# mrottmann/DDalphaAMG

Hardware: AMD Instinct MI355X
Metric: fine_wilson_clover_gflops (higher is better)
Workload: dtype f32; 1 GPU; fine Wilson-Clover apply (d_plus_clover), 32x32x32x32 local lattice per GPU, random SU(3) gauge, csw=1.0, anti-periodic T; parallelism=single, ranks=1

## Files before the change

ddalphaamg_amd/csrc/fine_op.h:

```cpp
#pragma once
#include "common.h"
#include "geometry.h"
#include "halo.h"

namespace ddamg {

template <typename T>
struct FineOpDev {
  const T* D;
  const T* clover;
  const T* clover_inv;
  const int* nb;
  int V;
  const T* halo;
  HaloDev hd;
  const int* tile_nb;
  const unsigned short* tnb;
  const unsigned char* parity;
  const T* Dc;
  const signed char* Dsgn;
  const T* cloverc;
};

template <typename T>
class FineOp {
 public:
  FineOp() = default;

  void upload(const Geometry& g, const double* D_ref, const double* clover_ref, const Knobs& knobs, hipStream_t st);
  void shift_diagonal(const double* clover64, double diff, hipStream_t st);
  const T* clover_field() const { return clover_; }
  void scale_clover(const double* base64, double scale_even, double scale_odd, hipStream_t st);
  void apply(T* eta, const T* phi, hipStream_t st) const;
  FineOpDev<T> dev() const { return FineOpDev<T>{D_, clover_, clover_inv_, nb_, V_, halo_.recv(), halo_.dev(), tile_nb_, tnb_, parity_, Dc_, Dsgn_, Cc_}; }
  bool links_compressed() const { return Dc_ != nullptr; }
  int V() const { return V_; }
  void apply_f32in(T* eta, const float* phi, hipStream_t st) const;
  void set_comm(Comm* c) { comm_ = c; }
  void halo_exchange(const T* v, hipStream_t st) const;
  void halo_begin(const T* v, hipStream_t st) const;
  void halo_finish(hipStream_t st) const;
  bool distributed() const { return halo_.active(); }
  void hop(T* out, const T* in, int par, hipStream_t st, int post = 0, const T* a = nullptr) const;
  void oo_inv(T* out, const T* in, hipStream_t st) const;
  void parity_select(T* out, const T* a, const T* b, int keep, hipStream_t st) const;

 private:
  DeviceBuffer<T> D_, clover_, clover_inv_;
  DeviceBuffer<int> nb_;
  DeviceBuffer<int> lex_;
  DeviceBuffer<unsigned char> parity_;
  DeviceBuffer<int> tile_nb_;
  T* Dc_ = nullptr;
  DeviceBuffer<T> Dc_store_;
  DeviceBuffer<signed char> Dsgn_;
  T* Cc_ = nullptr;
  DeviceBuffer<T> Cc_store_;
  DeviceBuffer<unsigned short> tnb_;
  int V_ = 0;
  mutable Halo<T> halo_;
  Comm* comm_ = nullptr;
};

template <>
void FineOp<double>::apply_f32in(double* eta, const float* phi, hipStream_t st) const;

#ifdef __HIPCC__
}
#include "dirac_device.h"
namespace ddamg {
template <typename T, int MU, bool CMP>
__device__ __forceinline__ void load_link(const FineOpDev<T>& op, size_t V, size_t s, T (&U)[18]) {
  if constexpr (!CMP) {
    load_site<T, 18>(op.D + (size_t)MU * 18 * V, V, s, U);
  } else {
    T r[12];
    load_site<T, 12>(op.Dc + (size_t)MU * 12 * V, V, s, r);
    const T sg = (T)2 * (T)op.Dsgn[(size_t)MU * V + s];
#pragma unroll
    for (int k = 0; k < 12; k++) U[k] = r[k];
#pragma unroll
    for (int k = 0; k < 3; k++) {
      const int k1 = (k + 1) % 3, k2 = (k + 2) % 3;
      const T cr = r[2 * k1] * r[6 + 2 * k2] - r[2 * k1 + 1] * r[6 + 2 * k2 + 1] - (r[2 * k2] * r[6 + 2 * k1] - r[2 * k2 + 1] * r[6 + 2 * k1 + 1]);
      const T ci = r[2 * k1] * r[6 + 2 * k2 + 1] + r[2 * k1 + 1] * r[6 + 2 * k2] - (r[2 * k2] * r[6 + 2 * k1 + 1] + r[2 * k2 + 1] * r[6 + 2 * k1]);
      U[12 + 2 * k] = sg * cr; U[12 + 2 * k + 1] = -sg * ci;
    }
  }
}

template <typename T, int MU>
__device__ __forceinline__ void halo_forward(const FineOpDev<T>& op, int slot, const T (&U)[18], T (&eta)[24]) {
  T h[12], g[12];
  load_site<T, 12>(op.halo + op.hd.off[MU], (size_t)op.hd.F[MU], (size_t)slot, h);
  su3_mul<T>(U, h, g);
  spin_reconstruct_sub<T, MU, -1>(g, eta);
}
template <typename T, int MU>
__device__ __forceinline__ void halo_backward(const FineOpDev<T>& op, int slot, T (&eta)[24]) {
  T g[12];
  load_site<T, 12>(op.halo + op.hd.off[4 + MU], (size_t)op.hd.F[MU], (size_t)slot, g);
  spin_reconstruct_sub<T, MU, +1>(g, eta);
}

#endif

template <typename T>
void vec_from_lex(T* dst, const double* src_lex_dev, const int* lex_of_site, int V, int ndof, hipStream_t st);
template <typename T>
void vec_to_lex(double* dst_lex_dev, const T* src, const int* lex_of_site, int V, int ndof, hipStream_t st);

template <typename T>
void aos_from_lex(T* dst, const double* src_lex_dev, const int* lex_of_site, int V, int ndof, hipStream_t st);
template <typename T>
void aos_to_lex(double* dst_lex_dev, const T* src, const int* lex_of_site, int V, int ndof, hipStream_t st);

}
```

ddalphaamg_amd/csrc/fine_op.hip:

```cpp
#include "fine_op.h"
#include "dirac_device.h"
#include <vector>
#include <complex>
#include <cstring>

#ifndef DDAMG_NT_CLOVER
#define DDAMG_NT_CLOVER true
#endif
#ifndef DDAMG_NT_STORE
#define DDAMG_NT_STORE true
#endif
namespace ddamg {

template <bool ARITH>
__device__ __forceinline__ int tile_neighbor(const int* __restrict__ nb, size_t V, size_t s, int d, int tile0, const uint4& q,
                                             const int* __restrict__ tile_nb, int ntiles_all) {
  if constexpr (!ARITH) {
    return nb[(size_t)d * V + s];
  } else {
    const unsigned w = (d >> 1) == 0 ? q.x : (d >> 1) == 1 ? q.y : (d >> 1) == 2 ? q.z : q.w;
    const unsigned e = (d & 1) ? (w >> 16) : (w & 0xffffu);
    const int li = (int)(e & 0x7fffu);
    if (!(e & 0x8000u)) return tile0 + li;
    const int tn = tile_nb[(size_t)d * ntiles_all + (tile0 >> 8)];
    return tn >= 0 ? tn * 256 + li : nb[(size_t)d * V + s];
  }
}

template <typename T, typename TIN, int NR>
__device__ __forceinline__ void load_site_as(const TIN* __restrict__ base, size_t V, size_t s, T (&out)[NR]) {
  if constexpr (sizeof(T) == sizeof(TIN)) load_site<T, NR>(reinterpret_cast<const T*>(base), V, s, out);
  else {
    TIN tmp[NR];
    load_site<TIN, NR>(base, V, s, tmp);
#pragma unroll
    for (int k = 0; k < NR; k++) out[k] = (T)tmp[k];
  }
}

template <typename T, int MU, bool ARITH, bool CMP, bool HB2, typename TIN = T, bool CCL = false>
__device__ __forceinline__ void tile_dir(const TIN* __restrict__ phi, const FineOpDev<T>& op, size_t s, bool live, int tile0, const uint4& q,
                                         const T (&p)[24], T (&e)[24], T* __restrict__ sp, T* __restrict__ hb) {
  const size_t V = op.V;
  const int t = threadIdx.x;
  T U[18];
  if (live) load_link<T, MU, CMP>(op, V, s, U);
  {
    T h[12], g[12];
    spin_project<T, MU, +1>(p, h);
    su3_mul_dag<T>(U, h, g);
#pragma unroll
    for (int c = 0; c < 12; c++) hb[c * 256 + t] = g[c];
  }
  if (live) {
    const int j = tile_neighbor<ARITH>(op.nb, V, s, MU, tile0, q, op.tile_nb, (int)(V >> 8));
    if (j >= 0) {
      T pn[24];
      if (j - tile0 >= 0 && j - tile0 < 256) {
#pragma unroll
        for (int c = 0; c < 24; c++) pn[c] = sp[c * 256 + (j - tile0)];
      } else {
        load_site_as<T, TIN, 24>(phi, V, j, pn);
      }
      hop_accumulate<T, MU, true>(U, pn, e);
    } else {
      halo_forward<T, MU>(op, -1 - j, U, e);
    }
  }
  __syncthreads();
  if (live) {
    const int j = tile_neighbor<ARITH>(op.nb, V, s, 4 + MU, tile0, q, op.tile_nb, (int)(V >> 8));
    if (j < 0) {
      halo_backward<T, MU>(op, -1 - j, e);
    } else if (j - tile0 >= 0 && j - tile0 < 256) {
      T g[12];
#pragma unroll
      for (int c = 0; c < 12; c++) g[c] = hb[c * 256 + (j - tile0)];
      spin_reconstruct_sub<T, MU, +1>(g, e);
    } else {
      T pn[24], Un[18];
      load_site_as<T, TIN, 24>(phi, V, j, pn);
      load_link<T, MU, CMP>(op, V, (size_t)j, Un);
      hop_accumulate<T, MU, false>(Un, pn, e);
    }
  }
  if constexpr (!HB2) __syncthreads();
}

template <typename T, bool ARITH, bool CMP = false, typename TIN = T, bool CCL = false>
__global__ __launch_bounds__(256, (sizeof(T) == 4 ? 3 : 2)) void dirac_apply_lds_kernel(T* __restrict__ eta, const TIN* __restrict__ phi, FineOpDev<T> op, int ntiles,
                                                                  const int* __restrict__ tile_list) {
  constexpr bool HB2 = sizeof(T) == 4;
  __shared__ T sp[24 * 256];
  __shared__ T hb[(HB2 ? 2 : 1) * 12 * 256];
  T* const hb1 = hb + (HB2 ? 12 * 256 : 0);
  int tile = blockIdx.x;
  if ((ntiles & 7) == 0) tile = (blockIdx.x & 7) * (ntiles >> 3) + (blockIdx.x >> 3);
  if (tile_list) tile = tile_list[tile];
  const size_t V = op.V;
  const int tile0 = tile * 256;
  const size_t s = (size_t)tile0 + threadIdx.x;
  const bool live = s < V;
  T p[24], e[24];
  uint4 q = make_uint4(0, 0, 0, 0);
  if constexpr (ARITH) q = reinterpret_cast<const uint4*>(op.tnb)[threadIdx.x];
  if (live) load_site_as<T, TIN, 24>(phi, V, s, p);
  else {
#pragma unroll
    for (int k = 0; k < 24; k++) p[k] = 0;
  }
#pragma unroll
  for (int c = 0; c < 24; c++) sp[c * 256 + threadIdx.x] = p[c];
  if (live) {
    if constexpr (CCL) {
      T cl[28];
      load_site<T, 28, DDAMG_NT_CLOVER>(op.cloverc, V, s, cl);
      herm6c_mul<T>(cl, p, e);
      load_site<T, 28, DDAMG_NT_CLOVER>(op.cloverc + (size_t)28 * V, V, s, cl);
      herm6c_mul<T>(cl, p + 12, e + 12);
    } else {
      T cl[36];
      load_site<T, 36, DDAMG_NT_CLOVER>(op.clover, V, s, cl);
      herm6_mul<T>(cl, p, e);
      load_site<T, 36, DDAMG_NT_CLOVER>(op.clover + (size_t)36 * V, V, s, cl);
      herm6_mul<T>(cl, p + 12, e + 12);
    }
  }
  __syncthreads();
  tile_dir<T, 0, ARITH, CMP, HB2, TIN, CCL>(phi, op, s, live, tile0, q, p, e, sp, hb);
  tile_dir<T, 1, ARITH, CMP, HB2, TIN, CCL>(phi, op, s, live, tile0, q, p, e, sp, hb1);
  tile_dir<T, 2, ARITH, CMP, HB2, TIN, CCL>(phi, op, s, live, tile0, q, p, e, sp, hb);
  tile_dir<T, 3, ARITH, CMP, HB2, TIN, CCL>(phi, op, s, live, tile0, q, p, e, sp, hb1);
  if (live) store_site<T, 24, DDAMG_NT_STORE>(eta, V, s, e);
}

template <typename T, int MU, bool ARITH>
__device__ __forceinline__ void tile_dir_parity(const T* __restrict__ phi, const FineOpDev<T>& op, size_t s, bool live, bool is_out, int tile0, const uint4& q,
                                                const T (&p)[24], T (&e)[24], T* __restrict__ sp, T* __restrict__ hb) {
  const size_t V = op.V;
  const int t = threadIdx.x;
  T U[18];
  if (live) load_site<T, 18>(op.D + (size_t)MU * 18 * V, V, s, U);
  if (live && !is_out) {
    T h[12], g[12];
    spin_project<T, MU, +1>(p, h);
    su3_mul_dag<T>(U, h, g);
#pragma unroll
    for (int c = 0; c < 12; c++) hb[c * 256 + t] = g[c];
  }
  if (live && is_out) {
    const int j = tile_neighbor<ARITH>(op.nb, V, s, MU, tile0, q, op.tile_nb, (int)(V >> 8));
    if (j >= 0) {
      T pn[24];
      if (j - tile0 >= 0 && j - tile0 < 256) {
#pragma unroll
        for (int c = 0; c < 24; c++) pn[c] = sp[c * 256 + (j - tile0)];
      } else {
        load_site<T, 24>(phi, V, j, pn);
      }
      hop_accumulate<T, MU, true>(U, pn, e);
    } else {
      halo_forward<T, MU>(op, -1 - j, U, e);
    }
  }
  __syncthreads();
  if (live && is_out) {
    const int j = tile_neighbor<ARITH>(op.nb, V, s, 4 + MU, tile0, q, op.tile_nb, (int)(V >> 8));
    if (j < 0) {
      halo_backward<T, MU>(op, -1 - j, e);
    } else if (j - tile0 >= 0 && j - tile0 < 256) {
      T g[12];
#pragma unroll
      for (int c = 0; c < 12; c++) g[c] = hb[c * 256 + (j - tile0)];
      spin_reconstruct_sub<T, MU, +1>(g, e);
    } else {
      T pn[24], Un[18];
      load_site<T, 24>(phi, V, j, pn);
      load_site<T, 18>(op.D + (size_t)MU * 18 * V, V, j, Un);
      hop_accumulate<T, MU, false>(Un, pn, e);
    }
  }
  __syncthreads();
}

template <typename T, bool ARITH>
__global__ __launch_bounds__(256, (sizeof(T) == 4 ? 3 : 2)) void dirac_hop_parity_kernel(T* __restrict__ eta, const T* __restrict__ phi, FineOpDev<T> op, int ntiles,
                                                                                         const int* __restrict__ tile_list, int par, int post,
                                                                                         const T* __restrict__ a) {
  __shared__ T sp[24 * 256];
  __shared__ T hb[12 * 256];
  int tile = blockIdx.x;
  if ((ntiles & 7) == 0) tile = (blockIdx.x & 7) * (ntiles >> 3) + (blockIdx.x >> 3);
  if (tile_list) tile = tile_list[tile];
  const size_t V = op.V;
  const int tile0 = tile * 256;
  const size_t s = (size_t)tile0 + threadIdx.x;
  const bool live = s < V;
  const bool is_out = live && op.parity[s] == par;
  T p[24], e[24];
  uint4 q = make_uint4(0, 0, 0, 0);
  if constexpr (ARITH) q = reinterpret_cast<const uint4*>(op.tnb)[threadIdx.x];
#pragma unroll
  for (int k = 0; k < 24; k++) { p[k] = 0; e[k] = 0; }
  if (live && !is_out) {
    load_site<T, 24>(phi, V, s, p);
#pragma unroll
    for (int c = 0; c < 24; c++) sp[c * 256 + threadIdx.x] = p[c];
  }
  __syncthreads();
  tile_dir_parity<T, 0, ARITH>(phi, op, s, live, is_out, tile0, q, p, e, sp, hb);
  tile_dir_parity<T, 1, ARITH>(phi, op, s, live, is_out, tile0, q, p, e, sp, hb);
  tile_dir_parity<T, 2, ARITH>(phi, op, s, live, is_out, tile0, q, p, e, sp, hb);
  tile_dir_parity<T, 3, ARITH>(phi, op, s, live, is_out, tile0, q, p, e, sp, hb);
  if (is_out) {
    if (post == 1) {
      T f[24], cl[36];
      load_site<T, 36>(op.clover_inv, V, s, cl);
      herm6_mul<T>(cl, e, f);
      load_site<T, 36>(op.clover_inv + (size_t)36 * V, V, s, cl);
      herm6_mul<T>(cl, e + 12, f + 12);
      store_site<T, 24>(eta, V, s, f);
    } else if (post == 2) {
      T pa[24], f[24], cl[36];
      load_site<T, 24>(a, V, s, pa);
      load_site<T, 36>(op.clover, V, s, cl);
      herm6_mul<T>(cl, pa, f);
      load_site<T, 36>(op.clover + (size_t)36 * V, V, s, cl);
      herm6_mul<T>(cl, pa + 12, f + 12);
#pragma unroll
      for (int k = 0; k < 24; k++) f[k] -= e[k];
      store_site<T, 24>(eta, V, s, f);
    } else {
      store_site<T, 24>(eta, V, s, e);
    }
  }
}

template <typename T, bool CCL>
static void launch_dirac_apply(T* eta, const T* phi, const FineOpDev<T>& op, int ntiles, const int* tile_list, hipStream_t st) {
  if (op.tnb && op.Dc) hipLaunchKernelGGL((dirac_apply_lds_kernel<T, true, true, T, CCL>), dim3(ntiles), dim3(256), 0, st, eta, phi, op, ntiles, tile_list);
  else if (op.tnb) hipLaunchKernelGGL((dirac_apply_lds_kernel<T, true, false, T, CCL>), dim3(ntiles), dim3(256), 0, st, eta, phi, op, ntiles, tile_list);
  else hipLaunchKernelGGL((dirac_apply_lds_kernel<T, false, false, T, CCL>), dim3(ntiles), dim3(256), 0, st, eta, phi, op, ntiles, tile_list);
}

template <typename T>
void FineOp<T>::apply(T* eta, const T* phi, hipStream_t st) const {
  DDAMG_REQUIRE(D_ != nullptr, "fine operator not uploaded");
  auto launch = [&](int ntiles, const int* tile_list) {
    if (ntiles == 0) return;
    if (Cc_) launch_dirac_apply<T, sizeof(T) == 4>(eta, phi, dev(), ntiles, tile_list, st);
    else launch_dirac_apply<T, false>(eta, phi, dev(), ntiles, tile_list, st);
    DDAMG_HIP_CHECK(hipGetLastError());
  };
  if (!halo_.active()) {
    launch((V_ + 255) / 256, nullptr);
    return;
  }
  halo_.pack(phi, D_, V_, st);
  halo_.exchange_begin(comm_, st);
  launch(halo_.n_interior(), halo_.interior_tiles());
  halo_.exchange_finish(comm_, st);
  launch(halo_.n_boundary(), halo_.boundary_tiles());
}

template <>
void FineOp<double>::apply_f32in(double* eta, const float* phi, hipStream_t st) const {
  DDAMG_REQUIRE(D_ != nullptr, "fine operator not uploaded");
  auto launch = [&](int ntiles, const int* tile_list) {
    if (ntiles == 0) return;
    if (tnb_ && Dc_) hipLaunchKernelGGL((dirac_apply_lds_kernel<double, true, true, float>), dim3(ntiles), dim3(256), 0, st, eta, phi, dev(), ntiles, tile_list);
    else if (tnb_) hipLaunchKernelGGL((dirac_apply_lds_kernel<double, true, false, float>), dim3(ntiles), dim3(256), 0, st, eta, phi, dev(), ntiles, tile_list);
    else hipLaunchKernelGGL((dirac_apply_lds_kernel<double, false, false, float>), dim3(ntiles), dim3(256), 0, st, eta, phi, dev(), ntiles, tile_list);
    DDAMG_HIP_CHECK(hipGetLastError());
  };
  if (!halo_.active()) { launch((V_ + 255) / 256, nullptr); return; }
  halo_.pack_f32in(phi, D_, V_, st);
  halo_.exchange_begin(comm_, st);
  launch(halo_.n_interior(), halo_.interior_tiles());
  halo_.exchange_finish(comm_, st);
  launch(halo_.n_boundary(), halo_.boundary_tiles());
}

template <typename T>
void FineOp<T>::hop(T* eta, const T* phi, int par, hipStream_t st, int post, const T* a) const {
  DDAMG_REQUIRE(post == 0 || post == 1 || (post == 2 && a != nullptr && a != eta), "hop: unknown epilogue");
  DDAMG_REQUIRE(D_ != nullptr, "fine operator not uploaded");
  auto launch = [&](int ntiles, const int* tile_list) {
    if (ntiles == 0) return;
    if (tnb_) hipLaunchKernelGGL((dirac_hop_parity_kernel<T, true>), dim3(ntiles), dim3(256), 0, st, eta, phi, dev(), ntiles, tile_list, par, post, a);
    else hipLaunchKernelGGL((dirac_hop_parity_kernel<T, false>), dim3(ntiles), dim3(256), 0, st, eta, phi, dev(), ntiles, tile_list, par, post, a);
    DDAMG_HIP_CHECK(hipGetLastError());
  };
  if (!halo_.active()) { launch((V_ + 255) / 256, nullptr); return; }
  halo_.pack(phi, D_, V_, st);
  halo_.exchange_begin(comm_, st);
  launch(halo_.n_interior(), halo_.interior_tiles());
  halo_.exchange_finish(comm_, st);
  launch(halo_.n_boundary(), halo_.boundary_tiles());
}

template <typename T>
void FineOp<T>::halo_begin(const T* v, hipStream_t st) const {
  if (!halo_.active()) return;
  halo_.pack(v, D_, V_, st);
  halo_.exchange_begin(comm_, st);
}
template <typename T>
void FineOp<T>::halo_finish(hipStream_t st) const {
  if (halo_.active()) halo_.exchange_finish(comm_, st);
}
template <typename T>
void FineOp<T>::halo_exchange(const T* v, hipStream_t st) const {
  halo_begin(v, st);
  halo_finish(st);
}

template <typename T>
__device__ __forceinline__ size_t soa_index_dev(int NR, size_t V, size_t s, int r) {
  constexpr int CH = Chunk<T>::CH;
  const int NF = NR / CH;
  if (r < NF * CH) return ((size_t)(r / CH) * V + s) * CH + (r % CH);
  const int TL = NR % CH;
  return (size_t)NF * V * CH + s * TL + (r - NF * CH);
}

__device__ __forceinline__ void gauss_jordan6(double (&mr)[6][12], double (&mi)[6][12]) {
  for (int col = 0; col < 6; col++) {
    int piv = col;
    double best = mr[col][col] * mr[col][col] + mi[col][col] * mi[col][col];
    for (int r = col + 1; r < 6; r++) {
      const double a2 = mr[r][col] * mr[r][col] + mi[r][col] * mi[r][col];
      if (a2 > best) { best = a2; piv = r; }
    }
    if (piv != col)
      for (int j = 0; j < 12; j++) {
        double t = mr[col][j]; mr[col][j] = mr[piv][j]; mr[piv][j] = t;
        t = mi[col][j]; mi[col][j] = mi[piv][j]; mi[piv][j] = t;
      }
    const double dr = mr[col][col] / best, di = -mi[col][col] / best;
    for (int j = 0; j < 12; j++) {
      const double xr = mr[col][j], xi = mi[col][j];
      mr[col][j] = xr * dr - xi * di; mi[col][j] = xr * di + xi * dr;
    }
    for (int r = 0; r < 6; r++) {
      if (r == col) continue;
      const double fr = mr[r][col], fi = mi[r][col];
      if (fr == 0.0 && fi == 0.0) continue;
      for (int j = 0; j < 12; j++) {
        mr[r][j] -= fr * mr[col][j] - fi * mi[col][j];
        mi[r][j] -= fr * mi[col][j] + fi * mr[col][j];
      }
    }
  }
}

__device__ __forceinline__ bool invert6_in_place(double (&ar)[6][6], double (&ai)[6][6]) {
  bool ok = true;
#pragma unroll
  for (int k = 0; k < 6; k++) {
    const double n2 = ar[k][k] * ar[k][k] + ai[k][k] * ai[k][k];
    ok = ok && n2 > 1e-24;
    const double pr = ar[k][k] / n2, pi = -ai[k][k] / n2;
#pragma unroll
    for (int j = 0; j < 6; j++)
      if (j != k) { const double xr = ar[k][j], xi = ai[k][j]; ar[k][j] = xr * pr - xi * pi; ai[k][j] = xr * pi + xi * pr; }
#pragma unroll
    for (int i = 0; i < 6; i++)
      if (i != k) {
        const double fr = ar[i][k], fi = ai[i][k];
#pragma unroll
        for (int j = 0; j < 6; j++)
          if (j != k) { ar[i][j] -= fr * ar[k][j] - fi * ai[k][j]; ai[i][j] -= fr * ai[k][j] + fi * ar[k][j]; }
        ar[i][k] = -(fr * pr - fi * pi); ai[i][k] = -(fr * pi + fi * pr);
      }
    ar[k][k] = pr; ai[k][k] = pi;
  }
  return ok;
}
__device__ __forceinline__ void invert_herm6(const double (&d)[6], const double (&ur)[15], const double (&ui)[15], double (&od)[6], double (&our)[15], double (&oui)[15]) {
  double ar[6][6], ai[6][6];
  {
    int k = 0;
#pragma unroll
    for (int i = 0; i < 6; i++) {
      ar[i][i] = d[i]; ai[i][i] = 0.0;
#pragma unroll
      for (int j = i + 1; j < 6; j++, k++) { ar[i][j] = ur[k]; ai[i][j] = ui[k]; ar[j][i] = ur[k]; ai[j][i] = -ui[k]; }
    }
  }
  if (!invert6_in_place(ar, ai)) {
    double mr[6][12], mi[6][12];
    for (int i = 0; i < 6; i++)
      for (int j = 0; j < 12; j++) { mr[i][j] = (j == 6 + i) ? 1.0 : 0.0; mi[i][j] = 0.0; }
    int k = 0;
    for (int i = 0; i < 6; i++) {
      mr[i][i] = d[i];
      for (int j = i + 1; j < 6; j++, k++) { mr[i][j] = ur[k]; mi[i][j] = ui[k]; mr[j][i] = ur[k]; mi[j][i] = -ui[k]; }
    }
    gauss_jordan6(mr, mi);
    k = 0;
    for (int i = 0; i < 6; i++) {
      od[i] = mr[i][6 + i];
      for (int j = i + 1; j < 6; j++, k++) { our[k] = mr[i][6 + j]; oui[k] = mi[i][6 + j]; }
    }
    return;
  }
  int k = 0;
#pragma unroll
  for (int i = 0; i < 6; i++) {
    od[i] = ar[i][i];
#pragma unroll
    for (int j = i + 1; j < 6; j++, k++) { our[k] = ar[i][j]; oui[k] = ai[i][j]; }
  }
}

template <typename T>
__device__ __forceinline__ bool compress_herm6(const double (&d)[6], const double (&ur)[15], const double (&ui)[15], T* __restrict__ out,
                                               size_t V, size_t s, int r0) {
  auto up = [](int i, int j) { return 5 * i - i * (i - 1) / 2 + j - i - 1; };
  double mx = 0, dev = 0, c = 0;
#pragma unroll
  for (int i = 0; i < 6; i++) mx = fmax(mx, fabs(d[i]));
#pragma unroll
  for (int k = 0; k < 15; k++) mx = fmax(mx, hypot(ur[k], ui[k]));
#pragma unroll
  for (int i = 0; i < 3; i++) {
    c += d[i] + d[3 + i];
    dev = fmax(dev, fabs(d[i] + d[3 + i] - (d[0] + d[3])));
#pragma unroll
    for (int j = i + 1; j < 3; j++) dev = fmax(dev, hypot(ur[up(i, j)] + ur[up(3 + i, 3 + j)], ui[up(i, j)] + ui[up(3 + i, 3 + j)]));
  }
  T v[28];
  v[0] = (T)(c / 6);
#pragma unroll
  for (int i = 0; i < 3; i++) v[1 + i] = (T)((d[i] - d[3 + i]) / 2);
#pragma unroll
  for (int i = 0; i < 3; i++)
#pragma unroll
    for (int j = i + 1; j < 3; j++) { v[4 + 2 * (i + j - 1)] = (T)ur[up(i, j)]; v[5 + 2 * (i + j - 1)] = (T)ui[up(i, j)]; }
#pragma unroll
  for (int i = 0; i < 3; i++)
#pragma unroll
    for (int j = 0; j < 3; j++) { v[10 + 2 * (3 * i + j)] = (T)ur[up(i, 3 + j)]; v[11 + 2 * (3 * i + j)] = (T)ui[up(i, 3 + j)]; }
#pragma unroll
  for (int r = 0; r < 28; r++) out[soa_index_dev<T>(56, V, s, r0 + r)] = v[r];
  return dev <= 1e-12 * mx;
}

template <typename T>
__global__ __launch_bounds__(128) void operator_layout_kernel(T* __restrict__ D, T* __restrict__ clover, T* __restrict__ clover_inv,
                                                              const double* __restrict__ D_lex, const double* __restrict__ clover_lex,
                                                              const int* __restrict__ lex_of_site, int V) {
  const size_t s = (size_t)blockIdx.x * 128 + threadIdx.x;
  if (s >= (size_t)V) return;
  const size_t lx = lex_of_site[s];
  for (int mu = 0; mu < 4; mu++)
    for (int r = 0; r < 18; r++)
      D[(size_t)mu * 18 * V + soa_index_dev<T>(18, V, s, r)] = (T)D_lex[(lx * 36 + mu * 9) * 2 + r];
  const double* c = clover_lex + lx * 42 * 2;
#pragma unroll
  for (int b = 0; b < 2; b++) {
    double d[6], ur[15], ui[15], od[6], our[15], oui[15];
#pragma unroll
    for (int i = 0; i < 6; i++) d[i] = c[2 * (6 * b + i)];
#pragma unroll
    for (int k = 0; k < 15; k++) { ur[k] = c[2 * (12 + 15 * b + k)]; ui[k] = c[2 * (12 + 15 * b + k) + 1]; }
    invert_herm6(d, ur, ui, od, our, oui);
    const int r0 = 36 * b;
#pragma unroll
    for (int i = 0; i < 6; i++) {
      clover[soa_index_dev<T>(72, V, s, r0 + i)] = (T)d[i];
      clover_inv[soa_index_dev<T>(72, V, s, r0 + i)] = (T)od[i];
    }
#pragma unroll
    for (int k = 0; k < 15; k++) {
      clover[soa_index_dev<T>(72, V, s, r0 + 6 + 2 * k)] = (T)ur[k];
      clover[soa_index_dev<T>(72, V, s, r0 + 6 + 2 * k + 1)] = (T)ui[k];
      clover_inv[soa_index_dev<T>(72, V, s, r0 + 6 + 2 * k)] = (T)our[k];
      clover_inv[soa_index_dev<T>(72, V, s, r0 + 6 + 2 * k + 1)] = (T)oui[k];
    }
  }
}

template <typename T>
__global__ __launch_bounds__(128) void clover_shift_kernel(T* clover, T* __restrict__ clover_inv, T* __restrict__ cloverc, const double* clover64, double diff,
                                                           int V) {
  const size_t s = (size_t)blockIdx.x * 128 + threadIdx.x;
  if (s >= (size_t)V) return;
#pragma unroll
  for (int b = 0; b < 2; b++) {
    double d[6], ur[15], ui[15], od[6], our[15], oui[15];
    const int r0 = 36 * b;
#pragma unroll
    for (int i = 0; i < 6; i++) d[i] = clover64[soa_index_dev<double>(72, V, s, r0 + i)] + diff;
#pragma unroll
    for (int k = 0; k < 15; k++) {
      ur[k] = clover64[soa_index_dev<double>(72, V, s, r0 + 6 + 2 * k)];
      ui[k] = clover64[soa_index_dev<double>(72, V, s, r0 + 6 + 2 * k + 1)];
    }
#pragma unroll
    for (int i = 0; i < 6; i++) clover[soa_index_dev<T>(72, V, s, r0 + i)] = (T)d[i];
    if (cloverc) (void)compress_herm6<T>(d, ur, ui, cloverc, V, s, 28 * b);
    invert_herm6(d, ur, ui, od, our, oui);
#pragma unroll
    for (int i = 0; i < 6; i++) clover_inv[soa_index_dev<T>(72, V, s, r0 + i)] = (T)od[i];
#pragma unroll
    for (int k = 0; k < 15; k++) {
      clover_inv[soa_index_dev<T>(72, V, s, r0 + 6 + 2 * k)] = (T)our[k];
      clover_inv[soa_index_dev<T>(72, V, s, r0 + 6 + 2 * k + 1)] = (T)oui[k];
    }
  }
}
template <typename T>
void FineOp<T>::shift_diagonal(const double* clover64, double diff, hipStream_t st) {
  DDAMG_REQUIRE(clover_ != nullptr && clover64 != nullptr, "shift_diagonal: no operator uploaded");
  hipLaunchKernelGGL(clover_shift_kernel<T>, dim3((unsigned)((V_ + 127) / 128)), dim3(128), 0, st, clover_, clover_inv_, Cc_, clover64, diff, (int)V_);
  DDAMG_HIP_CHECK(hipGetLastError());
}

template <typename T>
__global__ __launch_bounds__(128) void clover_scale_kernel(T* clover, T* __restrict__ clover_inv, T* __restrict__ cloverc, const double* base64,
                                                           const unsigned char* __restrict__ parity, double scale_even, double scale_odd, int V) {
  const size_t s = (size_t)blockIdx.x * 128 + threadIdx.x;
  if (s >= (size_t)V) return;
  const double f = parity[s] ? scale_odd : scale_even;
#pragma unroll
  for (int b = 0; b < 2; b++) {
    double d[6], ur[15], ui[15], od[6], our[15], oui[15];
    const int r0 = 36 * b;
#pragma unroll
    for (int i = 0; i < 6; i++) d[i] = f * base64[soa_index_dev<double>(72, V, s, r0 + i)];
#pragma unroll
    for (int k = 0; k < 15; k++) {
      ur[k] = f * base64[soa_index_dev<double>(72, V, s, r0 + 6 + 2 * k)];
      ui[k] = f * base64[soa_index_dev<double>(72, V, s, r0 + 6 + 2 * k + 1)];
    }
    if (cloverc) (void)compress_herm6<T>(d, ur, ui, cloverc, V, s, 28 * b);
    invert_herm6(d, ur, ui, od, our, oui);
#pragma unroll
    for (int i = 0; i < 6; i++) {
      clover[soa_index_dev<T>(72, V, s, r0 + i)] = (T)d[i];
      clover_inv[soa_index_dev<T>(72, V, s, r0 + i)] = (T)od[i];
    }
#pragma unroll
    for (int k = 0; k < 15; k++) {
      clover[soa_index_dev<T>(72, V, s, r0 + 6 + 2 * k)] = (T)ur[k];
      clover[soa_index_dev<T>(72, V, s, r0 + 6 + 2 * k + 1)] = (T)ui[k];
      clover_inv[soa_index_dev<T>(72, V, s, r0 + 6 + 2 * k)] = (T)our[k];
      clover_inv[soa_index_dev<T>(72, V, s, r0 + 6 + 2 * k + 1)] = (T)oui[k];
    }
  }
}
template <typename T>
void FineOp<T>::scale_clover(const double* base64, double scale_even, double scale_odd, hipStream_t st) {
  DDAMG_REQUIRE(clover_ != nullptr && base64 != nullptr && parity_ != nullptr, "scale_clover: no operator uploaded");
  DDAMG_REQUIRE((const void*)base64 != (const void*)clover_, "scale_clover: the unscaled copy must be a buffer of its own");
  hipLaunchKernelGGL(clover_scale_kernel<T>, dim3((unsigned)((V_ + 127) / 128)), dim3(128), 0, st, clover_, clover_inv_, Cc_, base64, parity_, scale_even, scale_odd, (int)V_);
  DDAMG_HIP_CHECK(hipGetLastError());
}

template <typename T>
__global__ __launch_bounds__(128) void link_compress_kernel(T* __restrict__ Dc, signed char* __restrict__ sgn, int* __restrict__ bad,
                                                            const double* __restrict__ D_lex, const int* __restrict__ lex_of_site, int V) {
  const size_t s = (size_t)blockIdx.x * 128 + threadIdx.x;
  if (s >= (size_t)V) return;
  const size_t lx = lex_of_site[s];
  for (int mu = 0; mu < 4; mu++) {
    const double* u = D_lex + (lx * 36 + mu * 9) * 2;
    double dev_p = 0, dev_m = 0, nrm = 0;
    for (int k = 0; k < 3; k++) {
      const int k1 = (k + 1) % 3, k2 = (k + 2) % 3;
      const double cr = u[2 * k1] * u[6 + 2 * k2] - u[2 * k1 + 1] * u[6 + 2 * k2 + 1] - (u[2 * k2] * u[6 + 2 * k1] - u[2 * k2 + 1] * u[6 + 2 * k1 + 1]);
      const double ci = u[2 * k1] * u[6 + 2 * k2 + 1] + u[2 * k1 + 1] * u[6 + 2 * k2] - (u[2 * k2] * u[6 + 2 * k1 + 1] + u[2 * k2 + 1] * u[6 + 2 * k1]);
      const double er = 2 * cr, ei = -2 * ci;
      dev_p += (u[12 + 2 * k] - er) * (u[12 + 2 * k] - er) + (u[12 + 2 * k + 1] - ei) * (u[12 + 2 * k + 1] - ei);
      dev_m += (u[12 + 2 * k] + er) * (u[12 + 2 * k] + er) + (u[12 + 2 * k + 1] + ei) * (u[12 + 2 * k + 1] + ei);
      nrm += u[12 + 2 * k] * u[12 + 2 * k] + u[12 + 2 * k + 1] * u[12 + 2 * k + 1];
    }
    const bool plus = dev_p <= dev_m;
    const double accept = sizeof(T) == 4 ? 1e-24 : 1e-28;
    if ((plus ? dev_p : dev_m) > accept * (nrm > 0 ? nrm : 1.0) || nrm == 0) atomicOr(bad, 1);
    sgn[(size_t)mu * V + s] = plus ? 1 : -1;
    for (int r = 0; r < 12; r++) Dc[(size_t)mu * 12 * V + soa_index_dev<T>(12, V, s, r)] = (T)u[r];
  }
}

template <typename T>
__global__ __launch_bounds__(128) void clover_compress_kernel(T* __restrict__ cloverc, int* __restrict__ bad, const double* __restrict__ clover_lex,
                                                              const int* __restrict__ lex_of_site, int V) {
  const size_t s = (size_t)blockIdx.x * 128 + threadIdx.x;
  if (s >= (size_t)V) return;
  const double* c = clover_lex + (size_t)lex_of_site[s] * 42 * 2;
  bool ok = true;
#pragma unroll
  for (int b = 0; b < 2; b++) {
    double d[6], ur[15], ui[15];
#pragma unroll
    for (int i = 0; i < 6; i++) d[i] = c[2 * (6 * b + i)];
#pragma unroll
    for (int k = 0; k < 15; k++) { ur[k] = c[2 * (12 + 15 * b + k)]; ui[k] = c[2 * (12 + 15 * b + k) + 1]; }
    ok = compress_herm6<T>(d, ur, ui, cloverc, V, s, 28 * b) && ok;
  }
  if (!ok) atomicOr(bad, 1);
}

template <typename T>
void FineOp<T>::upload(const Geometry& g, const double* D_ref, const double* clover_ref, const Knobs& knobs, hipStream_t st) {
  const size_t V = g.V;
  V_ = g.V;
  if (!D_) {
    D_.alloc(72 * V);
    clover_.alloc(72 * V);
    clover_inv_.alloc(72 * V);
    nb_.alloc(8 * V);
    lex_.alloc(V);
    DDAMG_HIP_CHECK(hipMemcpyAsync(lex_, g.lex_of_site.data(), sizeof(int) * V, hipMemcpyHostToDevice, st));
    std::vector<unsigned char> par(V);
    for (size_t i = 0; i < V; i++) par[i] = (unsigned char)g.parity[i];
    parity_.upload(par);
  }
  DeviceBuffer<double> dD, dC;
  dD.alloc(72 * V);
  dC.alloc(84 * V);
  DDAMG_HIP_CHECK(hipMemcpyAsync(dD, D_ref, sizeof(double) * 72 * V, hipMemcpyHostToDevice, st));
  DDAMG_HIP_CHECK(hipMemcpyAsync(dC, clover_ref, sizeof(double) * 84 * V, hipMemcpyHostToDevice, st));
  hipLaunchKernelGGL(operator_layout_kernel<T>, dim3((unsigned)((V + 127) / 128)), dim3(128), 0, st, D_, clover_, clover_inv_, dD, dC, lex_, (int)V);
  DDAMG_HIP_CHECK(hipGetLastError());
  Dc_ = nullptr;
  {
    if (knobs.link_compression && g.block_sites == 256) {
      if (!Dc_store_) {
        Dc_store_.alloc(48 * V);
        Dsgn_.alloc(4 * V, sizeof(int));
      }
      int* d_bad = reinterpret_cast<int*>(Dsgn_ + 4 * V);
      DDAMG_HIP_CHECK(hipMemsetAsync(d_bad, 0, sizeof(int), st));
      hipLaunchKernelGGL(link_compress_kernel<T>, dim3((unsigned)((V + 127) / 128)), dim3(128), 0, st, Dc_store_, Dsgn_, d_bad, dD, lex_, (int)V);
      DDAMG_HIP_CHECK(hipGetLastError());
      int bad = 1;
      DDAMG_HIP_CHECK(hipMemcpyAsync(&bad, d_bad, sizeof(int), hipMemcpyDeviceToHost, st));
      DDAMG_HIP_CHECK(hipStreamSynchronize(st));
      if (!bad) Dc_ = Dc_store_;
    }
  }
  Cc_ = nullptr;
  if constexpr (sizeof(T) == 4) {
    if (knobs.clover_compression) {
      if (!Cc_store_) Cc_store_.alloc(56 * V, sizeof(int));
      int* d_bad = reinterpret_cast<int*>(Cc_store_ + 56 * V);
      DDAMG_HIP_CHECK(hipMemsetAsync(d_bad, 0, sizeof(int), st));
      hipLaunchKernelGGL(clover_compress_kernel<T>, dim3((unsigned)((V + 127) / 128)), dim3(128), 0, st, Cc_store_, d_bad, dC, lex_, (int)V);
      DDAMG_HIP_CHECK(hipGetLastError());
      int bad = 1;
      DDAMG_HIP_CHECK(hipMemcpyAsync(&bad, d_bad, sizeof(int), hipMemcpyDeviceToHost, st));
      DDAMG_HIP_CHECK(hipStreamSynchronize(st));
      if (!bad) Cc_ = Cc_store_;
    }
  }
  DDAMG_HIP_CHECK(hipMemcpyAsync(nb_, g.nb.data(), sizeof(int) * 8 * V, hipMemcpyHostToDevice, st));
  if (g.block_sites == 256 && !tnb_) {
    tile_nb_.alloc(8 * g.num_blocks);
    tnb_.alloc(8 * 256);
    DDAMG_HIP_CHECK(hipMemcpyAsync(tile_nb_, g.block_nb.data(), sizeof(int) * 8 * g.num_blocks, hipMemcpyHostToDevice, st));
    DDAMG_HIP_CHECK(hipMemcpyAsync(tnb_, g.blk_wrap_nb.data(), sizeof(unsigned short) * 8 * 256, hipMemcpyHostToDevice, st));
  }
  DDAMG_HIP_CHECK(hipStreamSynchronize(st));
  dD.reset(); dC.reset();
  if (g.distributed() && !halo_.active()) halo_.init(g);
}

template <typename T>
__global__ __launch_bounds__(256) void oo_inv_kernel(T* __restrict__ out, const T* __restrict__ in, const T* __restrict__ clover_inv,
                                                     const unsigned char* __restrict__ parity, int V) {
  const size_t s = (size_t)blockIdx.x * 256 + threadIdx.x;
  if (s >= (size_t)V) return;
  T e[24];
  if (parity[s]) {
    T p[24], cl[36];
    load_site<T, 24>(in, V, s, p);
    load_site<T, 36>(clover_inv, V, s, cl);
    herm6_mul<T>(cl, p, e);
    load_site<T, 36>(clover_inv + (size_t)36 * V, V, s, cl);
    herm6_mul<T>(cl, p + 12, e + 12);
  } else {
#pragma unroll
    for (int k = 0; k < 24; k++) e[k] = 0;
  }
  store_site<T, 24>(out, V, s, e);
}
template <typename T>
__global__ __launch_bounds__(256) void parity_select_kernel(T* __restrict__ out, const T* __restrict__ a, const T* __restrict__ b,
                                                            const unsigned char* __restrict__ parity, int keep, int V) {
  const size_t s = (size_t)blockIdx.x * 256 + threadIdx.x;
  if (s >= (size_t)V) return;
  T e[24];
  if (parity[s] == keep) {
    load_site<T, 24>(a, V, s, e);
    if (b) {
      T f[24];
      load_site<T, 24>(b, V, s, f);
#pragma unroll
      for (int k = 0; k < 24; k++) e[k] -= f[k];
    }
  } else {
#pragma unroll
    for (int k = 0; k < 24; k++) e[k] = 0;
  }
  store_site<T, 24>(out, V, s, e);
}
template <typename T>
void FineOp<T>::oo_inv(T* out, const T* in, hipStream_t st) const {
  hipLaunchKernelGGL(oo_inv_kernel<T>, dim3((unsigned)((V_ + 255) / 256)), dim3(256), 0, st, out, in, clover_inv_, parity_, (int)V_);
  DDAMG_HIP_CHECK(hipGetLastError());
}
template <typename T>
void FineOp<T>::parity_select(T* out, const T* a, const T* b, int keep, hipStream_t st) const {
  hipLaunchKernelGGL(parity_select_kernel<T>, dim3((unsigned)((V_ + 255) / 256)), dim3(256), 0, st, out, a, b, parity_, keep, (int)V_);
  DDAMG_HIP_CHECK(hipGetLastError());
}

template <typename T>
__global__ void vec_from_lex_kernel(T* __restrict__ dst, const double* __restrict__ src, const int* __restrict__ lex_of_site, int V, int nreal) {
  constexpr int CH = Chunk<T>::CH;
  size_t i = (size_t)blockIdx.x * blockDim.x + threadIdx.x;
  size_t total = (size_t)V * nreal;
  if (i >= total) return;
  size_t k = i / ((size_t)V * CH);
  size_t rem = i - k * (size_t)V * CH;
  size_t s = rem / CH;
  int c = rem % CH;
  int r = (int)k * CH + c;
  dst[i] = (T)src[(size_t)lex_of_site[s] * nreal + r];
}
template <typename T>
__global__ void vec_to_lex_kernel(double* __restrict__ dst, const T* __restrict__ src, const int* __restrict__ lex_of_site, int V, int nreal) {
  constexpr int CH = Chunk<T>::CH;
  size_t i = (size_t)blockIdx.x * blockDim.x + threadIdx.x;
  size_t total = (size_t)V * nreal;
  if (i >= total) return;
  size_t k = i / ((size_t)V * CH);
  size_t rem = i - k * (size_t)V * CH;
  size_t s = rem / CH;
  int c = rem % CH;
  int r = (int)k * CH + c;
  dst[(size_t)lex_of_site[s] * nreal + r] = (double)src[i];
}

template <typename T>
void vec_from_lex(T* dst, const double* src, const int* lex_of_site, int V, int ndof, hipStream_t st) {
  int nreal = 2 * ndof;
  DDAMG_REQUIRE(nreal % Chunk<T>::CH == 0, "dof per site must fill whole 16-byte chunks");
  size_t total = (size_t)V * nreal;
  hipLaunchKernelGGL(vec_from_lex_kernel<T>, dim3((total + 255) / 256), dim3(256), 0, st, dst, src, lex_of_site, V, nreal);
  DDAMG_HIP_CHECK(hipGetLastError());
}
template <typename T>
void vec_to_lex(double* dst, const T* src, const int* lex_of_site, int V, int ndof, hipStream_t st) {
  int nreal = 2 * ndof;
  DDAMG_REQUIRE(nreal % Chunk<T>::CH == 0, "dof per site must fill whole 16-byte chunks");
  size_t total = (size_t)V * nreal;
  hipLaunchKernelGGL(vec_to_lex_kernel<T>, dim3((total + 255) / 256), dim3(256), 0, st, dst, src, lex_of_site, V, nreal);
  DDAMG_HIP_CHECK(hipGetLastError());
}

template <typename T, bool TO_LEX>
__global__ void aos_lex_kernel(T* __restrict__ v, double* __restrict__ lexv, const int* __restrict__ lex_of_site, int V, int nreal) {
  size_t i = (size_t)blockIdx.x * blockDim.x + threadIdx.x;
  if (i >= (size_t)V * nreal) return;
  const size_t s = i / nreal; const int r = (int)(i - s * nreal);
  if constexpr (TO_LEX) lexv[(size_t)lex_of_site[s] * nreal + r] = (double)v[i];
  else v[i] = (T)lexv[(size_t)lex_of_site[s] * nreal + r];
}
template <typename T>
void aos_from_lex(T* dst, const double* src, const int* lex_of_site, int V, int ndof, hipStream_t st) {
  size_t total = (size_t)V * 2 * ndof;
  hipLaunchKernelGGL((aos_lex_kernel<T, false>), dim3((total + 255) / 256), dim3(256), 0, st, dst, const_cast<double*>(src), lex_of_site, V, 2 * ndof);
  DDAMG_HIP_CHECK(hipGetLastError());
}
template <typename T>
void aos_to_lex(double* dst, const T* src, const int* lex_of_site, int V, int ndof, hipStream_t st) {
  size_t total = (size_t)V * 2 * ndof;
  hipLaunchKernelGGL((aos_lex_kernel<T, true>), dim3((total + 255) / 256), dim3(256), 0, st, const_cast<T*>(src), dst, lex_of_site, V, 2 * ndof);
  DDAMG_HIP_CHECK(hipGetLastError());
}
template void aos_from_lex<float>(float*, const double*, const int*, int, int, hipStream_t);
template void aos_from_lex<double>(double*, const double*, const int*, int, int, hipStream_t);
template void aos_to_lex<float>(double*, const float*, const int*, int, int, hipStream_t);
template void aos_to_lex<double>(double*, const double*, const int*, int, int, hipStream_t);

template class FineOp<float>;
template class FineOp<double>;
template void vec_from_lex<float>(float*, const double*, const int*, int, int, hipStream_t);
template void vec_from_lex<double>(double*, const double*, const int*, int, int, hipStream_t);
template void vec_to_lex<float>(double*, const float*, const int*, int, int, hipStream_t);
template void vec_to_lex<double>(double*, const double*, const int*, int, int, hipStream_t);

}
```

ddalphaamg_amd/csrc/knobs.h:

```cpp
#pragma once
#include <cstdlib>
#include <cstring>

namespace ddamg {

struct OptionalInt {
  bool set = false;
  int value = 0;
};

struct Knobs {
  bool link_compression = true;
  bool clover_compression = true;

  int sap_variant = 3;

  bool galerkin_unbatched = false;
  bool galerkin_full_fields = false;
  bool galerkin_store_columns = false;
  OptionalInt galerkin_slab_aggs;
  bool aggregate_dirac_gather = false;
  bool coarse_restrict_valu = false;

  bool bootstrap_unbatched = false;
  OptionalInt bootstrap_group;
  bool tv_gs_columnwise = false;

  bool gs_workgroup = false;
  bool coarse_gs_global = false;
  bool coarse_gs_workgroup_form = false;

  bool coarse_sap_unfused = false;
  int coarse_apply_once_min_sites = 2048;

  bool pipelined_arnoldi = false;
  bool single_allreduce_arnoldi = false;

  OptionalInt comm_cus;
  bool host_transport = false;

  bool setup_timing = false;

  static Knobs from_env() {
    const auto present = [](const char* name) { return getenv(name) != nullptr; };
    const auto unless_zero = [](const char* name) { const char* e = getenv(name); return !(e != nullptr && atoi(e) == 0); };
    const auto integer = [](const char* name) { const char* e = getenv(name); return e ? OptionalInt{true, atoi(e)} : OptionalInt{}; };
    Knobs k;
    k.link_compression = unless_zero("DDAMG_LINK_COMPRESSION");
    k.clover_compression = unless_zero("DDAMG_CLOVER_COMPRESSION");
    if (const OptionalInt v = integer("DDAMG_SAP_VARIANT"); v.set) k.sap_variant = v.value;
    k.galerkin_unbatched = present("DDAMG_GALERKIN_UNBATCHED");
    k.galerkin_full_fields = present("DDAMG_GALERKIN_FULL_FIELDS");
    k.galerkin_store_columns = present("DDAMG_GALERKIN_STORE_COLUMNS");
    k.galerkin_slab_aggs = integer("DDAMG_GALERKIN_SLAB_AGGS");
    k.aggregate_dirac_gather = present("DDAMG_AGGREGATE_DIRAC_GATHER");
    k.coarse_restrict_valu = present("DDAMG_COARSE_RESTRICT_VALU");
    k.bootstrap_unbatched = present("DDAMG_BOOTSTRAP_UNBATCHED");
    k.bootstrap_group = integer("DDAMG_BOOTSTRAP_GROUP");
    k.tv_gs_columnwise = present("DDAMG_TV_GS_COLUMNWISE");
    k.gs_workgroup = present("DDAMG_GS_WORKGROUP");
    k.coarse_gs_global = present("DDAMG_COARSE_GS_GLOBAL");
    if (const char* e = getenv("DDAMG_COARSE_GS_FORM")) k.coarse_gs_workgroup_form = e[0] == 'w';
    k.coarse_sap_unfused = present("DDAMG_COARSE_SAP_UNFUSED");
    if (const OptionalInt v = integer("DDAMG_COARSE_APPLY_ONCE_MIN_SITES"); v.set) k.coarse_apply_once_min_sites = v.value;
    k.pipelined_arnoldi = present("DDAMG_PIPELINED_ARNOLDI");
    k.single_allreduce_arnoldi = present("DDAMG_SINGLE_ALLREDUCE_ARNOLDI");
    k.comm_cus = integer("DDAMG_COMM_CUS");
    if (const char* e = getenv("DDAMG_HIP_TRANSPORT")) k.host_transport = strcmp(e, "host") == 0;
    k.setup_timing = present("DDAMG_SETUP_TIMING");
    return k;
  }
};

inline int comm_cus_for(const Knobs& knobs, int num_levels) { return knobs.comm_cus.set ? knobs.comm_cus.value : (num_levels <= 1 ? 24 : 0); }

inline bool poison_allocations() {
  static const bool on = getenv("DDAMG_POISON") != nullptr;
  return on;
}

}
```

Baseline: 15020 GFLOP/s.

## Compress fp32 fine gauge links to eight reals plus a tag

Result: no change. 14960 GFLOP/s, median of 2 (-0.4%).

```diff
diff --git a/ddalphaamg_amd/csrc/fine_op.h b/ddalphaamg_amd/csrc/fine_op.h
--- a/ddalphaamg_amd/csrc/fine_op.h
+++ b/ddalphaamg_amd/csrc/fine_op.h
@@ -20,7 +20,11 @@
   const T* Dc;
   const signed char* Dsgn;
   const T* cloverc;
+  const T* D8;
+  const unsigned short* D8tag;
 };
+
+enum LinkForm : int { LINK_FULL = 0, LINK_TWO_ROW = 1, LINK_EIGHT = 2 };
 
 template <typename T>
 class FineOp {
@@ -32,7 +36,8 @@
   const T* clover_field() const { return clover_; }
   void scale_clover(const double* base64, double scale_even, double scale_odd, hipStream_t st);
   void apply(T* eta, const T* phi, hipStream_t st) const;
-  FineOpDev<T> dev() const { return FineOpDev<T>{D_, clover_, clover_inv_, nb_, V_, halo_.recv(), halo_.dev(), tile_nb_, tnb_, parity_, Dc_, Dsgn_, Cc_}; }
+  FineOpDev<T> dev() const { return FineOpDev<T>{D_, clover_, clover_inv_, nb_, V_, halo_.recv(), halo_.dev(), tile_nb_, tnb_, parity_, Dc_, Dsgn_, Cc_, D8_, D8_ ? D8tag_.get() : nullptr}; }
+  bool links_eight() const { return D8_ != nullptr; }
   bool links_compressed() const { return Dc_ != nullptr; }
   int V() const { return V_; }
   void apply_f32in(T* eta, const float* phi, hipStream_t st) const;
@@ -56,6 +61,9 @@
   DeviceBuffer<signed char> Dsgn_;
   T* Cc_ = nullptr;
   DeviceBuffer<T> Cc_store_;
+  T* D8_ = nullptr;
+  DeviceBuffer<T> D8_store_;
+  DeviceBuffer<unsigned short> D8tag_;
   DeviceBuffer<unsigned short> tnb_;
   int V_ = 0;
   mutable Halo<T> halo_;
@@ -69,23 +77,67 @@
 }
 #include "dirac_device.h"
 namespace ddamg {
-template <typename T, int MU, bool CMP>
+template <typename T>
+__device__ __forceinline__ void link_third_row(const T sg, T (&U)[18]) {
+#pragma unroll
+  for (int k = 0; k < 3; k++) {
+    const int k1 = (k + 1) % 3, k2 = (k + 2) % 3;
+    const T cr = U[2 * k1] * U[6 + 2 * k2] - U[2 * k1 + 1] * U[6 + 2 * k2 + 1] - (U[2 * k2] * U[6 + 2 * k1] - U[2 * k2 + 1] * U[6 + 2 * k1 + 1]);
+    const T ci = U[2 * k1] * U[6 + 2 * k2 + 1] + U[2 * k1 + 1] * U[6 + 2 * k2] - (U[2 * k2] * U[6 + 2 * k1 + 1] + U[2 * k2 + 1] * U[6 + 2 * k1]);
+    U[12 + 2 * k] = sg * cr; U[12 + 2 * k + 1] = -sg * ci;
+  }
+}
+
+constexpr unsigned LINK8_D = 0, LINK8_DNEG = 3, LINK8_K = 4, LINK8_MINUS = 6, LINK8_DU = 8, LINK8_DUNEG = 10;
+
+template <typename T, int MU, int LF>
 __device__ __forceinline__ void load_link(const FineOpDev<T>& op, size_t V, size_t s, T (&U)[18]) {
-  if constexpr (!CMP) {
+  if constexpr (LF == LINK_FULL) {
     load_site<T, 18>(op.D + (size_t)MU * 18 * V, V, s, U);
-  } else {
+  } else if constexpr (LF == LINK_TWO_ROW) {
     T r[12];
     load_site<T, 12>(op.Dc + (size_t)MU * 12 * V, V, s, r);
     const T sg = (T)2 * (T)op.Dsgn[(size_t)MU * V + s];
 #pragma unroll
     for (int k = 0; k < 12; k++) U[k] = r[k];
+    link_third_row<T>(sg, U);
+  } else {
+    static_assert(sizeof(T) == 4, "the eight-real links exist in fp32 only");
+    T y[8];
+    load_site<T, 8>(op.D8 + (size_t)MU * 8 * V, V, s, y);
+    const unsigned tg = op.D8tag[(size_t)MU * V + s];
+    const unsigned d = (tg >> LINK8_D) & 7u, k = (tg >> LINK8_K) & 3u, du = (tg >> LINK8_DU) & 3u;
+    T x = sqrtf((T)1 - (y[0] * y[0] + y[1] * y[1] + y[2] * y[2] + y[3] * y[3] + y[4] * y[4]));
+    x = (tg >> LINK8_DNEG) & 1u ? -x : x;
+    T a[6];
+    a[0] = d == 0 ? x : y[0];
 #pragma unroll
-    for (int k = 0; k < 3; k++) {
-      const int k1 = (k + 1) % 3, k2 = (k + 2) % 3;
-      const T cr = r[2 * k1] * r[6 + 2 * k2] - r[2 * k1 + 1] * r[6 + 2 * k2 + 1] - (r[2 * k2] * r[6 + 2 * k1] - r[2 * k2 + 1] * r[6 + 2 * k1 + 1]);
-      const T ci = r[2 * k1] * r[6 + 2 * k2 + 1] + r[2 * k1 + 1] * r[6 + 2 * k2] - (r[2 * k2] * r[6 + 2 * k1 + 1] + r[2 * k2 + 1] * r[6 + 2 * k1]);
-      U[12 + 2 * k] = sg * cr; U[12 + 2 * k + 1] = -sg * ci;
-    }
+    for (int m = 1; m < 5; m++) a[m] = d == (unsigned)m ? x : (d < (unsigned)m ? y[m - 1] : y[m]);
+    a[5] = d == 5 ? x : y[4];
+    const T p0r = k == 0 ? a[0] : k == 1 ? a[2] : a[4], p0i = k == 0 ? a[1] : k == 1 ? a[3] : a[5];
+    const T p1r = k == 0 ? a[2] : k == 1 ? a[4] : a[0], p1i = k == 0 ? a[3] : k == 1 ? a[5] : a[1];
+    const T p2r = k == 0 ? a[4] : k == 1 ? a[0] : a[2], p2i = k == 0 ? a[5] : k == 1 ? a[1] : a[3];
+    T xu = sqrtf((T)1 - (y[5] * y[5] + y[6] * y[6] + y[7] * y[7]));
+    xu = (tg >> LINK8_DUNEG) & 1u ? -xu : xu;
+    const T u1r = du == 0 ? xu : y[5];
+    const T u1i = du == 1 ? xu : (du < 1 ? y[5] : y[6]);
+    const T u2r = du == 2 ? xu : (du < 2 ? y[6] : y[7]);
+    const T u2i = du == 3 ? xu : y[7];
+    const T r = sqrtf(p0r * p0r + p0i * p0i);
+    const T sr = p1r * u1r + p1i * u1i + p2r * u2r + p2i * u2i;
+    const T si = p1r * u1i - p1i * u1r + p2r * u2i - p2i * u2r;
+    const T f = (T)1 / ((T)1 + r), g = (T)-1 / r;
+    const T tr = sr * f, ti = si * f;
+    const T w1r = u1r - (p1r * tr - p1i * ti), w1i = u1i - (p1r * ti + p1i * tr);
+    const T w2r = u2r - (p2r * tr - p2i * ti), w2i = u2i - (p2r * ti + p2i * tr);
+    const T bkr = (sr * p0r - si * p0i) * g, bki = (sr * p0i + si * p0r) * g;
+    const T h = (tg >> LINK8_MINUS) & 1u ? (T)-0.5 : (T)0.5;
+#pragma unroll
+    for (int m = 0; m < 6; m++) U[m] = h * a[m];
+    U[6] = h * (k == 0 ? bkr : k == 1 ? w2r : w1r); U[7] = h * (k == 0 ? bki : k == 1 ? w2i : w1i);
+    U[8] = h * (k == 0 ? w1r : k == 1 ? bkr : w2r); U[9] = h * (k == 0 ? w1i : k == 1 ? bki : w2i);
+    U[10] = h * (k == 0 ? w2r : k == 1 ? w1r : bkr); U[11] = h * (k == 0 ? w2i : k == 1 ? w1i : bki);
+    link_third_row<T>((T)4 * h, U);
   }
 }
 
diff --git a/ddalphaamg_amd/csrc/fine_op.hip b/ddalphaamg_amd/csrc/fine_op.hip
--- a/ddalphaamg_amd/csrc/fine_op.hip
+++ b/ddalphaamg_amd/csrc/fine_op.hip
@@ -38,13 +38,13 @@
   }
 }
 
-template <typename T, int MU, bool ARITH, bool CMP, bool HB2, typename TIN = T, bool CCL = false>
+template <typename T, int MU, bool ARITH, int LF, bool HB2, typename TIN = T, bool CCL = false>
 __device__ __forceinline__ void tile_dir(const TIN* __restrict__ phi, const FineOpDev<T>& op, size_t s, bool live, int tile0, const uint4& q,
                                          const T (&p)[24], T (&e)[24], T* __restrict__ sp, T* __restrict__ hb) {
   const size_t V = op.V;
   const int t = threadIdx.x;
   T U[18];
-  if (live) load_link<T, MU, CMP>(op, V, s, U);
+  if (live) load_link<T, MU, LF>(op, V, s, U);
   {
     T h[12], g[12];
     spin_project<T, MU, +1>(p, h);
@@ -80,14 +80,14 @@
     } else {
       T pn[24], Un[18];
       load_site_as<T, TIN, 24>(phi, V, j, pn);
-      load_link<T, MU, CMP>(op, V, (size_t)j, Un);
+      load_link<T, MU, LF>(op, V, (size_t)j, Un);
       hop_accumulate<T, MU, false>(Un, pn, e);
     }
   }
   if constexpr (!HB2) __syncthreads();
 }
 
-template <typename T, bool ARITH, bool CMP = false, typename TIN = T, bool CCL = false>
+template <typename T, bool ARITH, int LF = LINK_FULL, typename TIN = T, bool CCL = false>
 __global__ __launch_bounds__(256, (sizeof(T) == 4 ? 3 : 2)) void dirac_apply_lds_kernel(T* __restrict__ eta, const TIN* __restrict__ phi, FineOpDev<T> op, int ntiles,
                                                                   const int* __restrict__ tile_list) {
   constexpr bool HB2 = sizeof(T) == 4;
@@ -127,10 +127,10 @@
     }
   }
   __syncthreads();
-  tile_dir<T, 0, ARITH, CMP, HB2, TIN, CCL>(phi, op, s, live, tile0, q, p, e, sp, hb);
-  tile_dir<T, 1, ARITH, CMP, HB2, TIN, CCL>(phi, op, s, live, tile0, q, p, e, sp, hb1);
-  tile_dir<T, 2, ARITH, CMP, HB2, TIN, CCL>(phi, op, s, live, tile0, q, p, e, sp, hb);
-  tile_dir<T, 3, ARITH, CMP, HB2, TIN, CCL>(phi, op, s, live, tile0, q, p, e, sp, hb1);
+  tile_dir<T, 0, ARITH, LF, HB2, TIN, CCL>(phi, op, s, live, tile0, q, p, e, sp, hb);
+  tile_dir<T, 1, ARITH, LF, HB2, TIN, CCL>(phi, op, s, live, tile0, q, p, e, sp, hb1);
+  tile_dir<T, 2, ARITH, LF, HB2, TIN, CCL>(phi, op, s, live, tile0, q, p, e, sp, hb);
+  tile_dir<T, 3, ARITH, LF, HB2, TIN, CCL>(phi, op, s, live, tile0, q, p, e, sp, hb1);
   if (live) store_site<T, 24, DDAMG_NT_STORE>(eta, V, s, e);
 }
 
@@ -238,9 +238,15 @@
 
 template <typename T, bool CCL>
 static void launch_dirac_apply(T* eta, const T* phi, const FineOpDev<T>& op, int ntiles, const int* tile_list, hipStream_t st) {
-  if (op.tnb && op.Dc) hipLaunchKernelGGL((dirac_apply_lds_kernel<T, true, true, T, CCL>), dim3(ntiles), dim3(256), 0, st, eta, phi, op, ntiles, tile_list);
-  else if (op.tnb) hipLaunchKernelGGL((dirac_apply_lds_kernel<T, true, false, T, CCL>), dim3(ntiles), dim3(256), 0, st, eta, phi, op, ntiles, tile_list);
-  else hipLaunchKernelGGL((dirac_apply_lds_kernel<T, false, false, T, CCL>), dim3(ntiles), dim3(256), 0, st, eta, phi, op, ntiles, tile_list);
+  if constexpr (sizeof(T) == 4) {
+    if (op.tnb && op.D8) {
+      hipLaunchKernelGGL((dirac_apply_lds_kernel<T, true, LINK_EIGHT, T, CCL>), dim3(ntiles), dim3(256), 0, st, eta, phi, op, ntiles, tile_list);
+      return;
+    }
+  }
+  if (op.tnb && op.Dc) hipLaunchKernelGGL((dirac_apply_lds_kernel<T, true, LINK_TWO_ROW, T, CCL>), dim3(ntiles), dim3(256), 0, st, eta, phi, op, ntiles, tile_list);
+  else if (op.tnb) hipLaunchKernelGGL((dirac_apply_lds_kernel<T, true, LINK_FULL, T, CCL>), dim3(ntiles), dim3(256), 0, st, eta, phi, op, ntiles, tile_list);
+  else hipLaunchKernelGGL((dirac_apply_lds_kernel<T, false, LINK_FULL, T, CCL>), dim3(ntiles), dim3(256), 0, st, eta, phi, op, ntiles, tile_list);
 }
 
 template <typename T>
@@ -268,9 +274,9 @@
   DDAMG_REQUIRE(D_ != nullptr, "fine operator not uploaded");
   auto launch = [&](int ntiles, const int* tile_list) {
     if (ntiles == 0) return;
-    if (tnb_ && Dc_) hipLaunchKernelGGL((dirac_apply_lds_kernel<double, true, true, float>), dim3(ntiles), dim3(256), 0, st, eta, phi, dev(), ntiles, tile_list);
-    else if (tnb_) hipLaunchKernelGGL((dirac_apply_lds_kernel<double, true, false, float>), dim3(ntiles), dim3(256), 0, st, eta, phi, dev(), ntiles, tile_list);
-    else hipLaunchKernelGGL((dirac_apply_lds_kernel<double, false, false, float>), dim3(ntiles), dim3(256), 0, st, eta, phi, dev(), ntiles, tile_list);
+    if (tnb_ && Dc_) hipLaunchKernelGGL((dirac_apply_lds_kernel<double, true, LINK_TWO_ROW, float>), dim3(ntiles), dim3(256), 0, st, eta, phi, dev(), ntiles, tile_list);
+    else if (tnb_) hipLaunchKernelGGL((dirac_apply_lds_kernel<double, true, LINK_FULL, float>), dim3(ntiles), dim3(256), 0, st, eta, phi, dev(), ntiles, tile_list);
+    else hipLaunchKernelGGL((dirac_apply_lds_kernel<double, false, LINK_FULL, float>), dim3(ntiles), dim3(256), 0, st, eta, phi, dev(), ntiles, tile_list);
     DDAMG_HIP_CHECK(hipGetLastError());
   };
   if (!halo_.active()) { launch((V_ + 255) / 256, nullptr); return; }
@@ -582,6 +588,43 @@
     if ((plus ? dev_p : dev_m) > accept * (nrm > 0 ? nrm : 1.0) || nrm == 0) atomicOr(bad, 1);
     sgn[(size_t)mu * V + s] = plus ? 1 : -1;
     for (int r = 0; r < 12; r++) Dc[(size_t)mu * 12 * V + soa_index_dev<T>(12, V, s, r)] = (T)u[r];
+  }
+}
+
+template <typename T>
+__global__ __launch_bounds__(128) void link_compress8_kernel(T* __restrict__ D8, unsigned short* __restrict__ tag, const signed char* __restrict__ sgn,
+                                                             const double* __restrict__ D_lex, const int* __restrict__ lex_of_site, int V) {
+  const size_t s = (size_t)blockIdx.x * 128 + threadIdx.x;
+  if (s >= (size_t)V) return;
+  const size_t lx = lex_of_site[s];
+  for (int mu = 0; mu < 4; mu++) {
+    const double* u = D_lex + (lx * 36 + mu * 9) * 2;
+    const bool minus = sgn[(size_t)mu * V + s] < 0;
+    const double two = minus ? -2.0 : 2.0;
+    double a[6], b[6], n2 = 0;
+    for (int m = 0; m < 6; m++) { a[m] = two * u[m]; b[m] = two * u[6 + m]; n2 += a[m] * a[m]; }
+    const double na = 1.0 / sqrt(n2);
+    for (int m = 0; m < 6; m++) a[m] *= na;
+    int d = 0, k = 0;
+    for (int m = 1; m < 6; m++) if (fabs(a[m]) > fabs(a[d])) d = m;
+    for (int m = 1; m < 3; m++) if (a[2 * m] * a[2 * m] + a[2 * m + 1] * a[2 * m + 1] > a[2 * k] * a[2 * k] + a[2 * k + 1] * a[2 * k + 1]) k = m;
+    const int i = (k + 1) % 3, j = (k + 2) % 3;
+    const double r = sqrt(a[2 * k] * a[2 * k] + a[2 * k + 1] * a[2 * k + 1]);
+    const double sr = a[2 * i] * b[2 * i] + a[2 * i + 1] * b[2 * i + 1] + a[2 * j] * b[2 * j] + a[2 * j + 1] * b[2 * j + 1];
+    const double si = a[2 * i] * b[2 * i + 1] - a[2 * i + 1] * b[2 * i] + a[2 * j] * b[2 * j + 1] - a[2 * j + 1] * b[2 * j];
+    const double q = 1.0 / (r * (1.0 + r));
+    double uu[4];
+    uu[0] = b[2 * i] + (a[2 * i] * sr - a[2 * i + 1] * si) * q; uu[1] = b[2 * i + 1] + (a[2 * i] * si + a[2 * i + 1] * sr) * q;
+    uu[2] = b[2 * j] + (a[2 * j] * sr - a[2 * j + 1] * si) * q; uu[3] = b[2 * j + 1] + (a[2 * j] * si + a[2 * j + 1] * sr) * q;
+    const double nu = 1.0 / sqrt(uu[0] * uu[0] + uu[1] * uu[1] + uu[2] * uu[2] + uu[3] * uu[3]);
+    int du = 0;
+    for (int m = 0; m < 4; m++) uu[m] *= nu;
+    for (int m = 1; m < 4; m++) if (fabs(uu[m]) > fabs(uu[du])) du = m;
+    T* out = D8 + (size_t)mu * 8 * V;
+    for (int m = 0, n = 0; m < 6; m++) if (m != d) out[soa_index_dev<T>(8, V, s, n++)] = (T)a[m];
+    for (int m = 0, n = 5; m < 4; m++) if (m != du) out[soa_index_dev<T>(8, V, s, n++)] = (T)uu[m];
+    tag[(size_t)mu * V + s] = (unsigned short)((unsigned)d << LINK8_D | (unsigned)(a[d] < 0) << LINK8_DNEG | (unsigned)k << LINK8_K |
+                                               (unsigned)minus << LINK8_MINUS | (unsigned)du << LINK8_DU | (unsigned)(uu[du] < 0) << LINK8_DUNEG);
   }
 }
 
@@ -643,6 +686,18 @@
       if (!bad) Dc_ = Dc_store_;
     }
   }
+  D8_ = nullptr;
+  if constexpr (sizeof(T) == 4) {
+    if (Dc_ && knobs.link_eight) {
+      if (!D8_store_) {
+        D8_store_.alloc(32 * V);
+        D8tag_.alloc(4 * V);
+      }
+      hipLaunchKernelGGL(link_compress8_kernel<T>, dim3((unsigned)((V + 127) / 128)), dim3(128), 0, st, D8_store_, D8tag_, Dsgn_, dD, lex_, (int)V);
+      DDAMG_HIP_CHECK(hipGetLastError());
+      D8_ = D8_store_;
+    }
+  }
   Cc_ = nullptr;
   if constexpr (sizeof(T) == 4) {
     if (knobs.clover_compression) {
diff --git a/ddalphaamg_amd/csrc/knobs.h b/ddalphaamg_amd/csrc/knobs.h
--- a/ddalphaamg_amd/csrc/knobs.h
+++ b/ddalphaamg_amd/csrc/knobs.h
@@ -12,6 +12,7 @@
 struct Knobs {
   bool link_compression = true;
   bool clover_compression = true;
+  bool link_eight = true;
 
   int sap_variant = 3;
 
@@ -48,6 +49,7 @@
     Knobs k;
     k.link_compression = unless_zero("DDAMG_LINK_COMPRESSION");
     k.clover_compression = unless_zero("DDAMG_CLOVER_COMPRESSION");
+    k.link_eight = unless_zero("DDAMG_LINK_EIGHT");
     if (const OptionalInt v = integer("DDAMG_SAP_VARIANT"); v.set) k.sap_variant = v.value;
     k.galerkin_unbatched = present("DDAMG_GALERKIN_UNBATCHED");
     k.galerkin_full_fields = present("DDAMG_GALERKIN_FULL_FIELDS");
```
